# datvo06/MSAU

Measured on AMD Instinct MI355X. Metric: chargrid tiles/sec (train fwd+bwd), 336x256x64 3-stage MSAU, higher is better.
Workload: dtype bf16; 1 GPU; configs[1]: one-hot chargrid 336x256x64, 3-stage MSAU (featRoot 8, 4 scales, res_depth 2), batch 16/GPU, fwd+masked-CE+bwd+clip+Adam; global_batch=16, parallelism=dp1, graph=False

## Files before the change

### include/msau_hip.h

```cpp
#ifndef MSAU_HIP_H
#define MSAU_HIP_H

#include <stdint.h>

#ifdef __cplusplus
extern "C" {
#endif

typedef enum { MSAU_F32 = 0, MSAU_BF16 = 1 } msau_dtype;

typedef enum {
    MSAU_OK = 0,
    MSAU_ERR_ARG = -1,
    MSAU_ERR_LDS = -2,
    MSAU_ERR_HIP = -3
} msau_status;

const char* msau_last_error(void);
int msau_version(void);
const char* msau_source_hash(void);
int msau_sizeof(int which);
int msau_lds_pixel_stride(int raw_bytes, int esz, int c8_per_chunk, int read_stride);
int msau_lds_wrow_stride(int nks, int esz);

// ... 120 lines not shown
    int32_t KH, KW, dil, pad_t, pad_l, stride;
    int32_t flags;
    const void* x1;
    const void* x2;
    const void* g;
    float* slabs;
    int32_t nslabs;
} msau_wgrad_desc;

typedef struct {
    int32_t cch, nchunks;
    int32_t kext;
    int32_t max_slabs;
    int64_t slab_bytes;
    int32_t lean;
    int32_t reserved;
} msau_wgrad_geom;

int msau_wgrad_geometry(int dtype, const msau_wgrad_desc* d, msau_wgrad_geom* out);
int msau_conv2d_wgrad(void* stream, int dtype, const msau_wgrad_desc* d);
int msau_wgrad_route(int dtype, const msau_wgrad_desc* d, int32_t info[8]);
int msau_conv2d_wgrad_groupable(int dtype, const msau_wgrad_desc* a, const msau_wgrad_desc* b);
int msau_conv2d_wgrad_group(void* stream, int dtype, const msau_wgrad_desc* const* ds, int n);

typedef struct {
    int64_t src_off;
    int64_t dst_off;
    int32_t kind;
    int32_t dim0, dim1;
    int32_t KH, KW;
    int32_t row_is_dim0;
    int32_t flip;
    int32_t row_off;
    int32_t rows_real;
    int32_t rows_pad;
    int32_t k1_real, k1_store, k2_real, k2_store;
    int32_t cch, nchunks, kchunk;
    int32_t dtype;
} msau_pack_entry;

int msau_pack_params(void* stream, const float* flat_params, void* pack_arena,
                     const msau_pack_entry* table_dev, int n_entries, int max_elems_per_entry);

typedef struct {
    int64_t slab_off;
    int64_t w_off;
// ... 282 lines not shown
```

### msau_amd/_lib.py

```python
from __future__ import annotations

import ctypes as C
import os

HERE = os.path.dirname(os.path.abspath(__file__))
LIB_PATH = os.environ.get("MSAU_HIP_LIB", os.path.join(HERE, "libmsau_hip.so"))

F32, BF16 = 0, 1
OPTIM_ADAM, OPTIM_RMSPROP, OPTIM_MOMENTUM, OPTIM_MAX_SKIP = 0, 1, 2, 8
COST_CE, COST_FOCAL, COST_DICE = 0, 1, 2

CONV_RELU_IN, CONV_RELU_OUT, CONV_ADD, CONV_ACCUM, CONV_MASK_A, CONV_MASK_B, CONV_HEAD, CONV_DOUT = 1, 2, 4, 8, 16, 32, 64, 128
CONV_LRN, CONV_POOL, CONV_IDS, CONV_OWNER, CONV_NCHW, CONV_WGRAD, CONV_ELU = 256, 512, 1024, 2048, 4096, 8192, 32768
CONV_EXTENT = 65536

i32, i64, vp, f32 = C.c_int32, C.c_int64, C.c_void_p, C.c_float


class ConvDesc(C.Structure):
    _fields_ = [(n, i32) for n in ("B", "Hin", "Win", "Hout", "Wout", "C1", "C2", "Cout", "KH", "KW", "dil",
                                   "pad_t", "pad_l", "stride", "ups", "flags")] + \
               [(n, vp) for n in ("x1", "x2", "wpack", "bias", "add", "mask_a", "mask_b", "y", "head_probs", "head_argmax")] + \
               [("head_classes", i32), ("flags2", i32), ("y2", vp), ("mask_b2", vp)] + \
               [("lrn_alpha_over_n", f32), ("lrn_beta", f32), ("lrn_k", f32), ("reserved0", i32), ("pool_y", vp), ("pool_idx", vp)] + \
# ... 117 lines not shown
    "msau_conv2d": (C.c_int, [vp, C.c_int, C.POINTER(ConvDesc)]),
    "msau_conv2d_rider_slabs": (C.c_int, [C.c_int, C.POINTER(ConvDesc)]),
    "msau_attn_proj_bwd": (C.c_int, [vp, C.c_int, C.POINTER(AttnProjBwdArgs)]),
    "msau_dgrad2_1x1": (C.c_int, [vp, C.c_int, C.POINTER(Dgrad2Args)]),
    "msau_conv2d_launch_info": (C.c_int, [C.c_int, C.POINTER(ConvDesc), C.POINTER(i32)]),
    "msau_conv_pair_applicable": (C.c_int, [C.c_int, C.POINTER(ConvPairDesc)]),
    "msau_conv_pair": (C.c_int, [vp, C.c_int, C.POINTER(ConvPairDesc)]),
    "msau_conv_pair_bits_bytes": (C.c_int64, [C.c_int, C.POINTER(ConvPairDesc)]),
    "msau_conv_pair_instance": (C.c_int, [C.c_int, C.POINTER(ConvPairDesc)]),
    "msau_conv_pair_wgrad_slabs": (C.c_int, [C.c_int, C.POINTER(ConvPairDesc)]),
    "msau_owner_slabs": (C.c_int, [C.POINTER(WgradDesc)]),
    "msau_comm_available": (C.c_int, []),
    "msau_comm_unique_id": (C.c_int, [vp, C.c_int]),
    "msau_comm_init": (C.c_int, [C.POINTER(vp), C.c_int, C.c_int, vp, C.c_int]),
    "msau_comm_destroy": (C.c_int, [vp]),
    "msau_allreduce_bucket": (C.c_int, [vp, vp, vp, C.c_int64]),
    "msau_run_ops_dp": (C.c_int, [vp, vp, vp, C.POINTER(Op), C.c_int, C.c_int]),
    "msau_reload_env": (None, []),
    "msau_wgrad_geometry": (C.c_int, [C.c_int, C.POINTER(WgradDesc), C.POINTER(WgradGeom)]),
    "msau_conv2d_wgrad": (C.c_int, [vp, C.c_int, C.POINTER(WgradDesc)]),
    "msau_wgrad_route": (C.c_int, [C.c_int, C.POINTER(WgradDesc), C.POINTER(i32)]),
    "msau_conv2d_wgrad_groupable": (C.c_int, [C.c_int, C.POINTER(WgradDesc), C.POINTER(WgradDesc)]),
    "msau_conv2d_wgrad_group": (C.c_int, [vp, C.c_int, C.POINTER(C.POINTER(WgradDesc)), C.c_int]),
    "msau_pack_params": (C.c_int, [vp, vp, vp, vp, C.c_int, C.c_int]),
    "msau_wgrad_reduce": (C.c_int, [vp, vp, vp, vp, C.c_int, C.c_int]),
    "msau_channel_sum": (C.c_int, [vp, C.c_int, vp, i64, C.c_int, vp, C.c_int]),
    "msau_nchw_to_nhwc": (C.c_int, [vp, C.c_int, vp, vp] + [C.c_int] * 5),
    "msau_nhwc_to_nchw": (C.c_int, [vp, C.c_int, vp, vp] + [C.c_int] * 5),
    "msau_nchw_grad_to_nhwc": (C.c_int, [vp, C.c_int, vp, vp] + [C.c_int] * 6),
    "msau_lrn_fwd": (C.c_int, [vp, C.c_int, vp, vp, i64, C.c_int, C.c_int, C.c_int, f32, f32, f32]),
    "msau_lrn_bwd": (C.c_int, [vp, C.c_int, vp, vp, vp, i64, C.c_int, C.c_int, C.c_int, f32, f32, f32]),
    "msau_maxpool2x2_fwd": (C.c_int, [vp, C.c_int, vp, vp, vp] + [C.c_int] * 4),
    "msau_maxpool2x2_bwd": (C.c_int, [vp, C.c_int, vp, vp, vp, vp] + [C.c_int] * 5),
    "msau_selfattn_fwd": (C.c_int, [vp, C.c_int, vp, vp, vp, vp, vp, vp] + [C.c_int] * 4),
    "msau_selfattn_bwd": (C.c_int, [vp, C.c_int, vp, vp, vp, vp, vp, vp, vp, vp, vp] + [C.c_int] * 4),
    "msau_maxpool2x2_bwd_ext": (C.c_int, [vp, C.c_int, vp, vp, vp, vp] + [C.c_int] * 5 + [vp]),
    "msau_selfattn_fwd_ext": (C.c_int, [vp, C.c_int, vp, vp, vp, vp, vp, vp] + [C.c_int] * 4 + [vp, C.c_int]),
    "msau_selfattn_bwd_ext": (C.c_int, [vp, C.c_int, vp, vp, vp, vp, vp, vp, vp, vp, vp] + [C.c_int] * 4 + [vp, C.c_int]),
    "msau_selfattn_route": (C.c_int, [C.c_int] * 4),
    "msau_extent_copy": (C.c_int, [vp, vp, vp] + [C.c_int] * 5 + [vp]),
    "msau_label_counts": (C.c_int, [vp, vp, vp, C.c_int, i64]),
    "msau_label_counts_split": (C.c_int, [vp, vp, vp, C.c_int, i64, C.c_int]),
    "msau_ce_ws_floats": (i64, [i64]),
    "msau_ce_multi_ws_floats": (i64, [i64]),
    "msau_masked_ce_multi": (C.c_int, [vp, C.c_int, vp, vp, vp, vp, vp, vp, vp, vp, C.c_int, i64, C.c_int, C.c_int, f32, C.c_int]),
    "msau_masked_ce": (C.c_int, [vp, C.c_int, vp, vp, vp, vp, vp, vp, C.c_int, i64, C.c_int, C.c_int, f32]),
# ... 180 lines not shown
```

### msau_amd/csrc/conv_wgrad.hip

```cpp
#include "msau_common.h"

namespace {

struct WGeom {
    int esz, taps, cch, nchunks, kreal, kextc, NKT, NKW, CTN, compact, slice;
    int TIH, TIW, PSx, PSg, x_bytes, g_bytes, tab_bytes, total;
};

inline int pix_stride(int c, int esz) {
    int ps = c * esz;
    if (((ps >> 4) & 1) == 0) ps += 16;
    return ps;
}

int wgrad_geom(int dtype, const msau_wgrad_desc* d, WGeom* out) {
    MSAU_CHECK_ARG(dtype == MSAU_F32 || dtype == MSAU_BF16, "wgrad: bad dtype");
    const int Cin = d->C1 + d->C2;
    MSAU_CHECK_ARG(Cin > 0 && Cin % 8 == 0 && d->Cout > 0 && d->Cout % 8 == 0 && d->Cout <= 1024, "wgrad: bad channels");
    MSAU_CHECK_ARG(d->KH >= 1 && d->KW >= 1 && d->KH <= 7 && d->KW <= 7 && d->dil >= 1 && (d->stride == 1 || d->stride == 2), "wgrad: bad kernel");
    WGeom g;
    g.esz = dtype == MSAU_F32 ? 4 : 2;
    g.taps = d->KH * d->KW;
    g.compact = d->stride == 1 && d->dil >= 16 && g.taps > 1;
    g.slice = g.esz == 4 ? (g.compact ? 32 : 64) : 128;
// ... 324 lines not shown
}

extern "C" int msau_conv2d_wgrad_groupable(int dtype, const msau_wgrad_desc* a, const msau_wgrad_desc* b) {
    if (!a || !b) return 0;
    WGeom g;
    WRoute r;
    return wgrad_route(dtype, a, &g, &r) == 0 && wgrad_groupable(r, a, b);
}

extern "C" int msau_conv2d_wgrad_group(void* stream, int dtype, const msau_wgrad_desc* const* ds, int n) {
    MSAU_CHECK_ARG(ds && n >= 1 && n <= 4, "wgrad_group: 1..4 launches");
    WGeom g;
    WRoute r;
    int rc = 0;
    for (int i = 0; i < n; ++i) {
        MSAU_CHECK_ARG(ds[i] && ds[i]->x1 && ds[i]->g && ds[i]->slabs && (ds[i]->C2 == 0 || ds[i]->x2), "wgrad_group: null pointer");
        if (i == 0 && n > 1) rc = wgrad_route(dtype, ds[0], &g, &r);
        MSAU_CHECK_ARG(i == 0 || (rc == 0 && wgrad_groupable(r, ds[0], ds[i])), "wgrad_group: launch %d differs in shape from launch 0", i);
    }
    if (n == 1) return msau_conv2d_wgrad(stream, dtype, ds[0]);
    if ((rc = wgrad_check_nslabs(ds[0], r))) return rc;
    return msau_wgrad_lean_launch(static_cast<hipStream_t>(stream), dtype, ds, n, &r);
}
```

### msau_amd/csrc/msau_common.h

```cpp
#pragma once
#include <hip/hip_runtime.h>
#include <stdint.h>
#include <stdio.h>
#include <stdarg.h>
#include "../../include/msau_hip.h"

typedef __bf16 bf16_t;
typedef __bf16 bf16x8 __attribute__((ext_vector_type(8)));
typedef __bf16 bf16x4 __attribute__((ext_vector_type(4)));
typedef float f32x4 __attribute__((ext_vector_type(4)));
typedef float f32x8 __attribute__((ext_vector_type(8)));

#define MSAU_LDS_LIMIT (160 * 1024)

int msau_set_error(int code, const char* fmt, ...);

constexpr int kFwd1 = MSAU_PAIR_RELU_IN | MSAU_PAIR_RELU_MID, kFwd2 = MSAU_CONV_ADD | MSAU_CONV_RELU_OUT;
constexpr int kBwd1 = MSAU_PAIR_MASK_MID, kBwd2 = MSAU_CONV_MASK_A | MSAU_CONV_ADD;
constexpr int kPairFwdRiders = MSAU_PAIR_COUPLE, kPairBwdRiders = MSAU_PAIR_LRN_BWD | MSAU_PAIR_WGRAD1 | MSAU_PAIR_DCOUPLE;
constexpr int kPairRiders = MSAU_PAIR_TILES | kPairFwdRiders | kPairBwdRiders;
enum { PAIR_NONE = 0, PAIR_TILE = 1, PAIR_ROWS = 2 };
enum { PAIR_FWD = 1, PAIR_BWD = 2 };
static inline int msau_pair_direction(const msau_conv_pair_desc* d) {
    const int f1 = d->flags1 & ~kPairRiders;
// ... 11 lines not shown
int msau_rowpair_case(int dtype, const msau_conv_pair_desc* d);
void msau_rowpair_split(const msau_conv_pair_desc* d, PairRoute* r);
int msau_rowpair_launch(hipStream_t s, const msau_conv_pair_desc* d, const PairRoute* r);
int msau_ownerconv_takes(int dtype, const msau_conv_desc* d);
int msau_ownerconv_fwd(hipStream_t s, int dtype, const msau_conv_desc* d);
int msau_rowconv_case(int dtype, const msau_conv_desc* d, int kchunk, int rows);
int msau_rowconv_launch(hipStream_t s, const msau_conv_desc* d, int kchunk, int rows, int inst);
int msau_rowconv_workgroups(const msau_conv_desc* d, int inst);
int msau_conv_chunked_case(int dtype, const msau_conv_desc* d, int cch, int nchunks, int CT);
int msau_conv_chunked_launch(hipStream_t s, int dtype, const msau_conv_desc* d, int kchunk, int nchunks, int CT, int which);
int msau_conv_lean_case(int dtype, const msau_conv_desc* d, int nchunks, int CT);
int msau_conv_lean_launch(hipStream_t s, int dtype, const msau_conv_desc* d, int kchunk, int CT, int which);
int msau_firstconv_takes(int dtype, const msau_conv_desc* d);
int msau_firstconv_launch(hipStream_t s, int dtype, const msau_conv_desc* d, int real_channels);
enum { WF_NONE = 0, WF_TILE = 1, WF_LEAN = 2, WF_SPECIAL = 3, WF_IN64 = 4, WF_IN64_IDS = 5, WF_ROWS = 6, WF_OWNER = 7 };
struct WRoute {
    int family, inst;
    int CTN, NKW, slices;
    int cch, nchunks, kextc;
    int tiles_x, tiles_y, ntiles;
};
int msau_wgrad_lean_case(int dtype, const msau_wgrad_desc* d, int cch, int kextc);
int msau_wgrad_lean_launch(hipStream_t s, int dtype, const msau_wgrad_desc* const* ds, int n, const WRoute* r);
int msau_rowwgrad_case(int dtype, const msau_wgrad_desc* d, int cch, int nchunks, int kextc);
int msau_rowwgrad_launch(hipStream_t s, const msau_wgrad_desc* d, int inst);
int msau_ownerconv_wgrad_case(int dtype, const msau_wgrad_desc* d, int cch, int nchunks, int kextc);
int msau_ownerconv_wgrad_launch(hipStream_t s, int dtype, const msau_wgrad_desc* d, const WRoute* r);

#define MSAU_CHECK_ARG(cond, ...)                                   \
    do {                                                            \
        if (!(cond)) return msau_set_error(MSAU_ERR_ARG, __VA_ARGS__); \
    } while (0)

#define MSAU_CHECK_LAUNCH(name)                                                         \
    do {                                                                                \
        hipError_t e__ = hipGetLastError();                                             \
        if (e__ != hipSuccess)                                                          \
            return msau_set_error(MSAU_ERR_HIP, "%s: %s", name, hipGetErrorString(e__)); \
    } while (0)

static inline int64_t cdiv64(int64_t a, int64_t b) { return (a + b - 1) / b; }
static inline int cdiv(int a, int b) { return (a + b - 1) / b; }
static inline int roundup(int a, int b) { return cdiv(a, b) * b; }

constexpr int kThreads = 256;

// ... 94 lines not shown
```

### msau_amd/csrc/sequence.hip

```cpp
#include "msau_common.h"

#include <cstdlib>
#include <utility>
#include <vector>

static int run_one_raw(void* stream, const msau_op& o, int i);

namespace {
struct ProbePair { hipEvent_t a, b; };
thread_local std::vector<ProbePair> g_probe_pool;
thread_local size_t g_probe_used = 0;
}

static int run_one(void* stream, const msau_op& o_in, int i) {
    if (!(o_in.kind & MSAU_OP_PROBE)) return run_one_raw(stream, o_in, i);
    msau_op o = o_in;
    o.kind &= ~MSAU_OP_PROBE;
    if (g_probe_used == g_probe_pool.size()) {
        ProbePair p;
        if (hipEventCreate(&p.a) != hipSuccess || hipEventCreate(&p.b) != hipSuccess)
            return msau_set_error(MSAU_ERR_HIP, "run_ops: cannot create probe events");
        g_probe_pool.push_back(p);
    }
    ProbePair& p = g_probe_pool[g_probe_used++];
// ... 65 lines not shown
        std::vector<hipEvent_t>& pl = sys ? pool_sys : pool;
        size_t& u = sys ? used_sys : used;
        if (u == pl.size()) {
            hipEvent_t e;
            hipError_t err = hipEventCreateWithFlags(&e, hipEventDisableTiming | (sys || fence_all ? 0u : hipEventDisableSystemFence));
            if (err != hipSuccess) return msau_set_error(MSAU_ERR_HIP, "run_ops_overlap: event: %s", hipGetErrorString(err));
            pl.push_back(e);
        }
        *ev = pl[u++];
        return 0;
    };
    auto next_event = [&](hipEvent_t* ev) -> int { return next_event_of(ev, false); };
    static const int fork_every = std::getenv("MSAU_FORK_EVERY") ? atoi(std::getenv("MSAU_FORK_EVERY")) : 6;
    std::vector<std::pair<msau_op, int>> pending;
    bool any_side = false;
    auto flush = [&]() -> int {
        if (pending.empty()) return 0;
        hipEvent_t ev;
        int rc = next_event(&ev);
        if (rc) return rc;
        if (hipEventRecord(ev, ms) != hipSuccess || hipStreamWaitEvent(ss, ev, 0) != hipSuccess)
            return msau_set_error(MSAU_ERR_HIP, "run_ops_overlap: fork failed");
        static const bool group_off = std::getenv("MSAU_WGRAD_GROUP") && std::getenv("MSAU_WGRAD_GROUP")[0] == '0';
        std::vector<char> done(pending.size(), 0);
        for (size_t i = 0; i < pending.size(); ++i) {
            if (done[i]) continue;
            const msau_op& o = pending[i].first;
            if (!group_off && o.kind == MSAU_OP_WGRAD) {
                const msau_wgrad_desc* ds[4] = {static_cast<const msau_wgrad_desc*>(o.args), nullptr, nullptr, nullptr};
                int n = 1;
                for (size_t j = i + 1; j < pending.size() && n < 4; ++j) {
                    const msau_op& p = pending[j].first;
                    if (done[j] || p.kind != MSAU_OP_WGRAD || p.dtype != o.dtype) continue;
                    if (!msau_conv2d_wgrad_groupable(o.dtype, ds[0], static_cast<const msau_wgrad_desc*>(p.args))) continue;
                    ds[n++] = static_cast<const msau_wgrad_desc*>(p.args);
                    done[j] = 1;
                }
                if (n > 1) {
                    rc = msau_conv2d_wgrad_group(side_stream, o.dtype, ds, n);
                    if (rc) return rc;
                    continue;
                }
            }
            rc = run_one(side_stream, o, pending[i].second);
            if (rc) return rc;
        }
        pending.clear();
        any_side = true;
        return 0;
    };
// ... 130 lines not shown
```

### msau_amd/csrc/wgrad_lean.hip

```cpp
#include "msau_common.h"
#include <cstdlib>

namespace {

struct WLeanArgs {
    msau_wgrad_desc d;
    int kextc, nchunks;
    int tiles_x, tiles_y, ntiles;
    unsigned mag_tx, mag_ty;
};

constexpr int kWGroup = 4;
struct WLeanMulti { WLeanArgs a[kWGroup]; };

#define WL_ABS 0x40000000
#ifndef MSAU_WPS_MAX
#define MSAU_WPS_MAX 10
#endif

typedef __attribute__((address_space(3))) bf16x4* lds_v4;

template <typename T, int C8, int CO8, int KS, int DIL = 1, int STRIDE = 1>
struct WLeanCfg {
    static constexpr int ESZ = (int)sizeof(T);
// ... 2 lines not shown
    static constexpr int QS = NMAP ? 4 : 8;
    static constexpr int HI = NMAP ? 8 : 4;
    static constexpr int PSX = NMAP ? lds_pixel_stride(C8 * 8 * ESZ, ESZ, C8, STRIDE) : (((C8 * 8 * ESZ / 16) % 2 == 0) ? C8 * 8 * ESZ + 16 : C8 * 8 * ESZ);
    static constexpr int PSG = NMAP ? lds_pixel_stride(CO8 * 8 * ESZ, ESZ, CO8, 1) : (((CO8 * 8 * ESZ / 16) % 2 == 0) ? CO8 * 8 * ESZ + 16 : CO8 * 8 * ESZ);
    static constexpr int KREAL = KS * KS * C8 * 8;
    static constexpr int KEXT = ((KREAL + 8 + 15) / 16) * 16;
    static constexpr int NKT = KEXT / 16;
    static constexpr int NKW = (NKT + 3) / 4;
    static constexpr int CTN = (CO8 + 1) / 2;
    static constexpr int X_BYTES = ((TI * TI * PSX + 15) / 16) * 16;
    static constexpr int G_BYTES = 256 * PSG;
    static constexpr bool PS = ESZ == 2 && NKT * CTN <= MSAU_WPS_MAX;
#ifndef MSAU_WGRAD_W2
#define MSAU_WGRAD_W2 1
#endif
    static constexpr bool W2 = MSAU_WGRAD_W2 && ESZ == 2 && !PS;
    static constexpr int NTH = W2 ? 512 : 256;
    static constexpr int RED_BYTES = PS ? 4 * NKT * CTN * 1024 : 0;
    static constexpr int TILE_BYTES = X_BYTES + G_BYTES + 64;
    static constexpr int LDS = TILE_BYTES > RED_BYTES ? TILE_BYTES : RED_BYTES;
};

template <typename T, int C8, int CO8, int KS, int DIL = 1, int STRIDE = 1>
__global__ __launch_bounds__((WLeanCfg<T, C8, CO8, KS, DIL, STRIDE>::NTH)) void wgrad_lean_kernel(const WLeanMulti m) {
    const WLeanArgs a = m.a[blockIdx.z];
    using Cfg = WLeanCfg<T, C8, CO8, KS, DIL, STRIDE>;
    typedef typename Vec8<T>::type V8;
    constexpr int ESZ = Cfg::ESZ, TI = Cfg::TI, PSX = Cfg::PSX, PSG = Cfg::PSG, NKT = Cfg::NKT, NKW = Cfg::NKW, CTN = Cfg::CTN;
    extern __shared__ __align__(16) unsigned char smem[];
    unsigned char* lds_x = smem;
    unsigned char* lds_g = smem + Cfg::X_BYTES;
    constexpr int ONES = Cfg::X_BYTES + Cfg::G_BYTES;

    const msau_wgrad_desc& d = a.d;
    constexpr int NTH = Cfg::NTH;
    const int tid = threadIdx.x, lane = tid & 63;
    const int wave = __builtin_amdgcn_readfirstlane((tid >> 6) & 3);
    const int wset = Cfg::W2 ? __builtin_amdgcn_readfirstlane(tid >> 8) : 0;
    const int li = lane & 15, lg = lane >> 4;
    const int chunk = blockIdx.y;
    const bool relu_in = d.flags & MSAU_CONV_RELU_IN;

    const int c0 = chunk * C8 * 8;
    const bool second = d.C2 != 0 && c0 >= d.C1;
    const char* xsrc = static_cast<const char*>(second ? d.x2 : d.x1);
    const int Cx = second ? d.C2 : d.C1;
    const int cb = (second ? c0 - d.C1 : c0) * ESZ;
    const int in_px = Cx * ESZ, in_row = d.Win * in_px;
    const int g_px = d.Cout * ESZ, g_row = d.Wout * g_px;

    if (tid < 8) reinterpret_cast<T*>(smem + ONES)[tid] = (T)(tid == 0 ? 1.0f : 0.0f);

    constexpr bool PS = Cfg::PS;
    constexpr int NACC = PS ? NKT : NKW;
    int coloff[NACC];
#pragma unroll
    for (int i = 0; i < NACC; ++i) {
        const int nkt = PS ? i : wave + 4 * i;
        const int k = nkt * 16 + (sizeof(T) == 2 ? (li & 3) * 4 : (li >> 2) * 4);
        int off;
        if (!PS && nkt >= NKT) off = WL_ABS | (ONES + 4 * ESZ);
        else if (k < Cfg::KREAL) {
            const int tap = k / (C8 * 8), c = k - tap * (C8 * 8);
// ... 29 lines not shown
                const int idx = tid + it * NTH;
                xr[it] = zero8<T>();
                if ((it + 1) * NTH <= NITEMS || idx < NITEMS) {
                    const int pix = idx / C8, cg = idx - pix * C8;
                    const int iy = pix / TI, ix = pix - iy * TI;
                    const int vy = vy0 + iy, vx = vx0 + ix;
                    if ((unsigned)vy < (unsigned)d.Hin && (unsigned)vx < (unsigned)d.Win)
                        xr[it] = *reinterpret_cast<const V8*>(base + (unsigned)(vy * in_row + vx * in_px + cg * 8 * ESZ));
                }
            }
        }
        {
            const char* base = static_cast<const char*>(d.g) + (long long)b * d.Hout * g_row;
#pragma unroll
            for (int it = 0; it < NITG; ++it) {
                const int idx = tid + it * NTH;
                const int m = idx / CO8, cg = idx - m * CO8;
                const int oy = oy0 + (m >> 4), ox = ox0 + (m & 15);
                gr[it] = zero8<T>();
                if (idx < 256 * CO8 && oy < d.Hout && ox < d.Wout) gr[it] = *reinterpret_cast<const V8*>(base + (unsigned)(oy * g_row + ox * g_px + cg * 8 * ESZ));
            }
        }
    };
    if (PIPE && (int)blockIdx.x < a.ntiles) issue_loads(blockIdx.x);

    for (int tile = blockIdx.x; tile < a.ntiles; tile += gridDim.x) {
        __syncthreads();
        if (!PIPE) issue_loads(tile);
        {
            constexpr int NITEMS = TI * TI * C8;
#pragma unroll
            for (int it = 0; it < NITX; ++it) {
                const int idx = tid + it * NTH;
                if ((it + 1) * NTH <= NITEMS || idx < NITEMS) {
                    const int pix = idx / C8, cg = idx - pix * C8;
                    V8 v = xr[it];
                    if (relu_in) v = relu8<T>(v);
                    *reinterpret_cast<V8*>(lds_x + pix * PSX + cg * 8 * ESZ) = v;
                }
            }
#pragma unroll
            for (int it = 0; it < NITG; ++it) {
                const int idx = tid + it * NTH;
                const int m = idx / CO8, cg = idx - m * CO8;
                if (idx < 256 * CO8) *reinterpret_cast<V8*>(lds_g + m * PSG + cg * 8 * ESZ) = gr[it];
            }
        }
        __syncthreads();
        if (PIPE && tile + (int)gridDim.x < a.ntiles) issue_loads(tile + gridDim.x);

        if constexpr (PS) {
            const int q = li >> 2, p = li & 3;
#pragma unroll
            for (int bb = 0; bb < 2; ++bb) {
                const int blk = wave * 2 + bb;
                const int row = blk * 2 + (lg >> 1), col = (lg & 1) * Cfg::QS + q;
                const unsigned char* ga = lds_g + (row * 16 + col) * PSG + 4 * p * 2;
                bf16x8 afrag[CTN];
#pragma unroll
                for (int ct = 0; ct < CTN; ++ct) {
                    bf16x4 lo = __builtin_amdgcn_ds_read_tr16_b64_v4bf16((lds_v4)(ga + ct * 32));
                    bf16x4 hi = __builtin_amdgcn_ds_read_tr16_b64_v4bf16((lds_v4)(ga + Cfg::HI * PSG + ct * 32));
                    afrag[ct] = __builtin_shufflevector(lo, hi, 0, 1, 2, 3, 4, 5, 6, 7);
                }
                const int pb0 = (row * STRIDE * TI + col * STRIDE) * PSX;
#pragma unroll
                for (int i = 0; i < NKT; ++i) {
                    const int e = coloff[i];
                    const bool abs_ok = (i + 1) * 16 > Cfg::KREAL;
                    const int o0 = (abs_ok && (e & WL_ABS)) ? (e & ~WL_ABS) : pb0 + e;
                    const int o1 = (abs_ok && (e & WL_ABS)) ? (e & ~WL_ABS) : pb0 + Cfg::HI * STRIDE * PSX + e;
                    bf16x4 lo = __builtin_amdgcn_ds_read_tr16_b64_v4bf16((lds_v4)(smem + o0));
// ... 33 lines not shown
                    for (int ct = 0; ct < CTN; ++ct)
                        acc[i][ct] = __builtin_amdgcn_mfma_f32_16x16x32_bf16(afrag[ct], bfrag, acc[i][ct], 0, 0, 0);
                }
            }
        } else {
            for (int step = 0; step < 64; ++step) {
                const int m = step * 4 + lg;
                float afrag[CTN];
#pragma unroll
                for (int ct = 0; ct < CTN; ++ct) afrag[ct] = *reinterpret_cast<const float*>(lds_g + m * PSG + (ct * 16 + li) * 4);
                const int pb = ((m >> 4) * STRIDE * TI + (m & 15) * STRIDE) * PSX;
#pragma unroll
                for (int i = 0; i < NKW; ++i) {
                    const int e = coloff[i];
                    const float bv = *reinterpret_cast<const float*>(smem + ((e & WL_ABS) ? (e & ~WL_ABS) : pb + e));
#pragma unroll
                    for (int ct = 0; ct < CTN; ++ct)
                        acc[i][ct] = __builtin_amdgcn_mfma_f32_16x16x4f32(afrag[ct], bv, acc[i][ct], 0, 0, 0);
                }
            }
        }
    }

    float* slab = d.slabs + ((size_t)blockIdx.x * a.nchunks + chunk) * d.Cout * a.kextc;
    if constexpr (PS) {
        __syncthreads();
        f32x4* red = reinterpret_cast<f32x4*>(smem);
#pragma unroll
        for (int i = 0; i < NKT; ++i)
#pragma unroll
            for (int ct = 0; ct < CTN; ++ct) red[((wave * NKT + i) * CTN + ct) * 64 + lane] = acc[i][ct];
        __syncthreads();
#pragma unroll
        for (int ii = 0; ii < NKW; ++ii) {
            const int nkt = wave + 4 * ii;
            if (nkt >= NKT) continue;
#pragma unroll
            for (int ct = 0; ct < CTN; ++ct) {
                f32x4 v = red[((0 * NKT + nkt) * CTN + ct) * 64 + lane];
#pragma unroll
                for (int w = 1; w < 4; ++w) v += red[((w * NKT + nkt) * CTN + ct) * 64 + lane];
#pragma unroll
                for (int j = 0; j < 4; ++j) {
                    const int co = ct * 16 + lg * 4 + j;
                    if (co < d.Cout) slab[(size_t)co * a.kextc + nkt * 16 + li] = v[j];
                }
            }
        }
        return;
    }
    if constexpr (Cfg::W2) {
        constexpr int PER = Cfg::TILE_BYTES / (4 * CTN * 1024) < 1 ? 1 : Cfg::TILE_BYTES / (4 * CTN * 1024);
        f32x4* red = reinterpret_cast<f32x4*>(smem);
        for (int i0 = 0; i0 < NKW; i0 += PER) {
            __syncthreads();
            if (wset == 1) {
#pragma unroll
                for (int i = 0; i < NKW; ++i)
                    if (i >= i0 && i < i0 + PER)
#pragma unroll
                        for (int ct = 0; ct < CTN; ++ct) red[((wave * PER + (i - i0)) * CTN + ct) * 64 + lane] = acc[i][ct];
            }
            __syncthreads();
            if (wset == 0) {
#pragma unroll
                for (int i = 0; i < NKW; ++i)
                    if (i >= i0 && i < i0 + PER)
#pragma unroll
                        for (int ct = 0; ct < CTN; ++ct) acc[i][ct] += red[((wave * PER + (i - i0)) * CTN + ct) * 64 + lane];
            }
        }
        if (wset == 1) return;
    }
#pragma unroll
    for (int i = 0; i < NKW; ++i) {
        const int nkt = wave + 4 * i;
        if (nkt >= NKT) continue;
#pragma unroll
        for (int ct = 0; ct < CTN; ++ct)
#pragma unroll
            for (int j = 0; j < 4; ++j) {
                const int co = ct * 16 + lg * 4 + j;
                if (co < d.Cout) slab[(size_t)co * a.kextc + nkt * 16 + li] = acc[i][ct][j];
            }
    }
}


struct WIn64 {
    static constexpr int PSX = 64 * 2 + 32, PSG = 8 * 2 + 32, TG = 18;
    static constexpr int X_BYTES = 256 * PSX, G_BYTES = TG * TG * PSG;
    static constexpr int ZERO = X_BYTES + G_BYTES;
    static constexpr int TILE_BYTES = ZERO + 64;
    static constexpr int RED_BYTES = 4 * 10 * 1024;
    static constexpr int LDS = TILE_BYTES > RED_BYTES ? TILE_BYTES : RED_BYTES;
};

template <bool IDS>
__global__ __launch_bounds__(256) void wgrad_in64_kernel(const WLeanArgs a) {
    typedef bf16_t T;
    typedef Vec8<T>::type V8;
    constexpr int PSX = WIn64::PSX, PSG = WIn64::PSG, TG = WIn64::TG;
    extern __shared__ __align__(16) unsigned char smem[];
    unsigned char* lds_x = smem;
    unsigned char* lds_g = smem + WIn64::X_BYTES;
    const msau_wgrad_desc& d = a.d;
    const int tid = threadIdx.x, lane = tid & 63;
    const int wave = __builtin_amdgcn_readfirstlane(tid >> 6);
// ... 199 lines not shown
#define WLEAN_TABLE(X)                                                                                                          \
    WLEAN_SHAPES(X, 1) WLEAN_SHAPES(X, 3) X(WF_LEAN, 8, 8, 1, 1, 1, 1) X(WF_LEAN, 8, 8, 3, 1, 1, 0) X(WF_LEAN, 1, 1, 4, 1, 1, 1)   \
    X(WF_SPECIAL, 1, 2, 3, 2, 1, 1) X(WF_SPECIAL, 2, 4, 3, 4, 1, 1) X(WF_SPECIAL, 4, 8, 3, 8, 1, 0)                             \
    X(WF_SPECIAL, 1, 2, 3, 1, 2, 1) X(WF_SPECIAL, 2, 4, 3, 1, 2, 1) X(WF_SPECIAL, 4, 8, 3, 1, 2, 0)                             \
    X(WF_IN64, 8, 1, 3, 1, 1, 0)

template <typename T>
int wlean_instance(int id, int kextc, hipStream_t s, const WLeanMulti* m, int n) {
    switch (id) {
#define WLEAN_ROW(FAM, C8, CO8, KS, DIL, STRIDE, F32)                                                                           \
        case wlean_id(FAM, C8, CO8, KS, DIL, STRIDE):                                                                           \
            if constexpr (FAM == WF_IN64) {                                                                                     \
                if (sizeof(T) == 2 && kextc == 592) return m ? launch_wgrad_in64(s, m->a[0]) : 1;                                \
            } else if constexpr (F32 || sizeof(T) == 2) {                                                                       \
                if (WLeanCfg<T, C8, CO8, KS, DIL, STRIDE>::KEXT == kextc) return m ? launch_wlean<T, C8, CO8, KS, DIL, STRIDE>(s, *m, n) : 1; \
            }                                                                                                                   \
            break;
        WLEAN_TABLE(WLEAN_ROW)
#undef WLEAN_ROW
    }
    return m ? msau_set_error(MSAU_ERR_ARG, "wgrad_lean: no instance %#x with k extent %d", id, kextc) : 0;
}

bool wlean_in64(int dtype, const msau_wgrad_desc* d, int cch) {
    static const bool in64_off = std::getenv("MSAU_WGRAD_IN64") && std::getenv("MSAU_WGRAD_IN64")[0] == '0';
    return !in64_off && dtype == MSAU_BF16 && d->stride == 1 && d->dil == 1 && d->KH == 3 && cch == 64 && d->Cout == 8 &&
           d->pad_t <= 2 && d->pad_l <= 2;
}

}

int msau_wgrad_lean_case(int dtype, const msau_wgrad_desc* d, int cch, int kextc) {
    if (d->KH != d->KW || d->dil > 8) return 0;
    const bool special = d->stride != 1 || d->dil != 1;
    if (special) {
        if (d->C2 || cch != d->C1 || d->pad_t != d->dil || d->pad_l != d->dil) return 0;
    } else {
        if (d->Hin != d->Hout || d->Win != d->Wout || d->pad_t < 0 || d->pad_l < 0 || d->pad_t >= d->KH || d->pad_l >= d->KW) return 0;
    }
    const int esz = dtype == MSAU_F32 ? 4 : 2;
    if ((int64_t)d->Hin * d->Win * (d->C1 > d->C2 ? d->C1 : d->C2) * esz >= (1ll << 31)) return 0;
    if ((int64_t)d->Hout * d->Wout * d->Cout * esz >= (1ll << 31)) return 0;
    const int tx = cdiv(d->Wout, 16), ty = cdiv(d->Hout, 16);
    if ((int64_t)d->B * tx * ty >= (1 << 20) || tx >= 4096 || ty >= 4096) return 0;
    const int fam = special ? WF_SPECIAL : wlean_in64(dtype, d, cch) ? WF_IN64 : WF_LEAN;
    const int id = wlean_id(fam, cch / 8, d->Cout / 8, d->KH, d->dil, d->stride);
    return (dtype == MSAU_F32 ? wlean_instance<float>(id, kextc, nullptr, nullptr, 0) : wlean_instance<bf16_t>(id, kextc, nullptr, nullptr, 0)) ? id : 0;
}

int msau_wgrad_lean_launch(hipStream_t s, int dtype, const msau_wgrad_desc* const* ds, int n, const WRoute* r) {
    MSAU_CHECK_ARG(n >= 1 && n <= ((r->inst & 7) == WF_IN64 ? 1 : kWGroup), "wgrad_lean: %d launches in one grid", n);
    WLeanMulti m;
    for (int i = 0; i < n; ++i) {
        WLeanArgs& a = m.a[i];
        a.d = *ds[i];
        a.kextc = r->kextc; a.nchunks = r->nchunks;
        a.tiles_x = r->tiles_x; a.tiles_y = r->tiles_y; a.ntiles = r->ntiles;
        a.mag_tx = (unsigned)((0x100000000ull + a.tiles_x - 1) / a.tiles_x);
        a.mag_ty = (unsigned)((0x100000000ull + a.tiles_y - 1) / a.tiles_y);
    }
    for (int i = n; i < kWGroup; ++i) m.a[i] = m.a[0];
    return dtype == MSAU_F32 ? wlean_instance<float>(r->inst, r->kextc, s, &m, n) : wlean_instance<bf16_t>(r->inst, r->kextc, s, &m, n);
}
```

Measured before the change: 5776 tiles/s.

## Batch wgrad lean layers of one occupancy class into a single persistent task kernel

Adds a task-list kernel that runs weight-gradient computations for up to 16 lean-route layers in one launch. Layers are grouped by an occupancy class derived from register and LDS limits, then sorted by per-slab work length, and each block dispatches to the right templated body through a switch. The goal is to cut per-layer launch overhead and fill the GPU better when each small layer alone uses fewer blocks than there are CUs. In exchange the kernel argument struct is larger, the dynamic LDS is sized for the largest member, and the switch may affect code size and register allocation.

```diff
diff --git a/include/msau_hip.h b/include/msau_hip.h
--- a/include/msau_hip.h
+++ b/include/msau_hip.h
@@ -166,6 +166,8 @@
 int msau_wgrad_route(int dtype, const msau_wgrad_desc* d, int32_t info[8]);
 int msau_conv2d_wgrad_groupable(int dtype, const msau_wgrad_desc* a, const msau_wgrad_desc* b);
 int msau_conv2d_wgrad_group(void* stream, int dtype, const msau_wgrad_desc* const* ds, int n);
+int msau_conv2d_wgrad_task_class(int dtype, const msau_wgrad_desc* d);
+int msau_conv2d_wgrad_tasks(void* stream, int dtype, const msau_wgrad_desc* const* ds, int n);
 
 typedef struct {
     int64_t src_off;
diff --git a/msau_amd/_lib.py b/msau_amd/_lib.py
--- a/msau_amd/_lib.py
+++ b/msau_amd/_lib.py
@@ -163,6 +163,8 @@
     "msau_wgrad_route": (C.c_int, [C.c_int, C.POINTER(WgradDesc), C.POINTER(i32)]),
     "msau_conv2d_wgrad_groupable": (C.c_int, [C.c_int, C.POINTER(WgradDesc), C.POINTER(WgradDesc)]),
     "msau_conv2d_wgrad_group": (C.c_int, [vp, C.c_int, C.POINTER(C.POINTER(WgradDesc)), C.c_int]),
+    "msau_conv2d_wgrad_task_class": (C.c_int, [C.c_int, C.POINTER(WgradDesc)]),
+    "msau_conv2d_wgrad_tasks": (C.c_int, [vp, C.c_int, C.POINTER(C.POINTER(WgradDesc)), C.c_int]),
     "msau_pack_params": (C.c_int, [vp, vp, vp, vp, C.c_int, C.c_int]),
     "msau_wgrad_reduce": (C.c_int, [vp, vp, vp, vp, C.c_int, C.c_int]),
     "msau_channel_sum": (C.c_int, [vp, C.c_int, vp, i64, C.c_int, vp, C.c_int]),
diff --git a/msau_amd/csrc/conv_wgrad.hip b/msau_amd/csrc/conv_wgrad.hip
--- a/msau_amd/csrc/conv_wgrad.hip
+++ b/msau_amd/csrc/conv_wgrad.hip
@@ -370,3 +370,50 @@
     if ((rc = wgrad_check_nslabs(ds[0], r))) return rc;
     return msau_wgrad_lean_launch(static_cast<hipStream_t>(stream), dtype, ds, n, &r);
 }
+
+
+namespace {
+int device_cus() {
+    static const int cus = [] {
+        int dev = 0, n = 0;
+        if (hipGetDevice(&dev) != hipSuccess || hipDeviceGetAttribute(&n, hipDeviceAttributeMultiprocessorCount, dev) != hipSuccess || n <= 0) {
+            (void)hipGetLastError();
+            n = 256;
+        }
+        return n;
+    }();
+    return cus;
+}
+
+int wgrad_task_class(int dtype, const msau_wgrad_desc* d, const WRoute& r) {
+    if (r.family != WF_LEAN && r.family != WF_SPECIAL) return 0;
+    if (d->nslabs < 1 || (int64_t)d->nslabs * r.nchunks > device_cus()) return 0;
+    return msau_wgrad_lean_task_class(dtype, &r);
+}
+}
+
+extern "C" int msau_conv2d_wgrad_task_class(int dtype, const msau_wgrad_desc* d) {
+    if (!d) return 0;
+    WGeom g;
+    WRoute r;
+    return wgrad_route(dtype, d, &g, &r) == 0 ? wgrad_task_class(dtype, d, r) : 0;
+}
+
+extern "C" int msau_conv2d_wgrad_tasks(void* stream, int dtype, const msau_wgrad_desc* const* ds, int n) {
+    MSAU_CHECK_ARG(ds && n >= 2 && n <= 16, "wgrad_tasks: 2..16 launches");
+    WGeom g;
+    WRoute rs[16];
+    int cls = 0;
+    for (int i = 0; i < n; ++i) {
+        const msau_wgrad_desc* d = ds[i];
+        MSAU_CHECK_ARG(d && d->x1 && d->g && d->slabs && (d->C2 == 0 || d->x2), "wgrad_tasks: null pointer");
+        int rc = wgrad_route(dtype, d, &g, &rs[i]);
+        if (rc) return rc;
+        if ((rc = wgrad_check_nslabs(d, rs[i]))) return rc;
+        const int c = wgrad_task_class(dtype, d, rs[i]);
+        MSAU_CHECK_ARG(c != 0, "wgrad_tasks: launch %d has no task class", i);
+        MSAU_CHECK_ARG(i == 0 || c == cls, "wgrad_tasks: launch %d is of task class %d, launch 0 of %d", i, c, cls);
+        cls = c;
+    }
+    return msau_wgrad_lean_tasks(static_cast<hipStream_t>(stream), dtype, cls, ds, rs, n);
+}
diff --git a/msau_amd/csrc/msau_common.h b/msau_amd/csrc/msau_common.h
--- a/msau_amd/csrc/msau_common.h
+++ b/msau_amd/csrc/msau_common.h
@@ -57,6 +57,8 @@
 };
 int msau_wgrad_lean_case(int dtype, const msau_wgrad_desc* d, int cch, int kextc);
 int msau_wgrad_lean_launch(hipStream_t s, int dtype, const msau_wgrad_desc* const* ds, int n, const WRoute* r);
+int msau_wgrad_lean_task_class(int dtype, const WRoute* r);
+int msau_wgrad_lean_tasks(hipStream_t s, int dtype, int cls, const msau_wgrad_desc* const* ds, const WRoute* rs, int n);
 int msau_rowwgrad_case(int dtype, const msau_wgrad_desc* d, int cch, int nchunks, int kextc);
 int msau_rowwgrad_launch(hipStream_t s, const msau_wgrad_desc* d, int inst);
 int msau_ownerconv_wgrad_case(int dtype, const msau_wgrad_desc* d, int cch, int nchunks, int kextc);
diff --git a/msau_amd/csrc/sequence.hip b/msau_amd/csrc/sequence.hip
--- a/msau_amd/csrc/sequence.hip
+++ b/msau_amd/csrc/sequence.hip
@@ -111,10 +111,32 @@
         if (hipEventRecord(ev, ms) != hipSuccess || hipStreamWaitEvent(ss, ev, 0) != hipSuccess)
             return msau_set_error(MSAU_ERR_HIP, "run_ops_overlap: fork failed");
         static const bool group_off = std::getenv("MSAU_WGRAD_GROUP") && std::getenv("MSAU_WGRAD_GROUP")[0] == '0';
+        static const bool tasks_off = std::getenv("MSAU_WGRAD_TASKS") && std::getenv("MSAU_WGRAD_TASKS")[0] == '0';
         std::vector<char> done(pending.size(), 0);
+        std::vector<int> cls(pending.size(), 0);
+        if (!tasks_off && pending.size() > 1)
+            for (size_t i = 0; i < pending.size(); ++i)
+                if (pending[i].first.kind == MSAU_OP_WGRAD)
+                    cls[i] = msau_conv2d_wgrad_task_class(pending[i].first.dtype, static_cast<const msau_wgrad_desc*>(pending[i].first.args));
         for (size_t i = 0; i < pending.size(); ++i) {
             if (done[i]) continue;
             const msau_op& o = pending[i].first;
+            if (cls[i]) {
+                const msau_wgrad_desc* ts[16] = {static_cast<const msau_wgrad_desc*>(o.args)};
+                size_t at[16];
+                int n = 1;
+                for (size_t j = i + 1; j < pending.size() && n < 16; ++j) {
+                    if (done[j] || cls[j] != cls[i] || pending[j].first.dtype != o.dtype) continue;
+                    at[n] = j;
+                    ts[n++] = static_cast<const msau_wgrad_desc*>(pending[j].first.args);
+                }
+                if (n > 1) {
+                    rc = msau_conv2d_wgrad_tasks(side_stream, o.dtype, ts, n);
+                    if (rc) return rc;
+                    for (int k = 1; k < n; ++k) done[at[k]] = 1;
+                    continue;
+                }
+            }
             if (!group_off && o.kind == MSAU_OP_WGRAD) {
                 const msau_wgrad_desc* ds[4] = {static_cast<const msau_wgrad_desc*>(o.args), nullptr, nullptr, nullptr};
                 int n = 1;
diff --git a/msau_amd/csrc/wgrad_lean.hip b/msau_amd/csrc/wgrad_lean.hip
--- a/msau_amd/csrc/wgrad_lean.hip
+++ b/msau_amd/csrc/wgrad_lean.hip
@@ -48,8 +48,7 @@
 };
 
 template <typename T, int C8, int CO8, int KS, int DIL = 1, int STRIDE = 1>
-__global__ __launch_bounds__((WLeanCfg<T, C8, CO8, KS, DIL, STRIDE>::NTH)) void wgrad_lean_kernel(const WLeanMulti m) {
-    const WLeanArgs a = m.a[blockIdx.z];
+__device__ __forceinline__ void wgrad_lean_body(const WLeanArgs& a, const unsigned slab_i, const unsigned nslab, const int chunk) {
     using Cfg = WLeanCfg<T, C8, CO8, KS, DIL, STRIDE>;
     typedef typename Vec8<T>::type V8;
     constexpr int ESZ = Cfg::ESZ, TI = Cfg::TI, PSX = Cfg::PSX, PSG = Cfg::PSG, NKT = Cfg::NKT, NKW = Cfg::NKW, CTN = Cfg::CTN;
@@ -64,7 +63,6 @@
     const int wave = __builtin_amdgcn_readfirstlane((tid >> 6) & 3);
     const int wset = Cfg::W2 ? __builtin_amdgcn_readfirstlane(tid >> 8) : 0;
     const int li = lane & 15, lg = lane >> 4;
-    const int chunk = blockIdx.y;
     const bool relu_in = d.flags & MSAU_CONV_RELU_IN;
 
     const int c0 = chunk * C8 * 8;
@@ -140,9 +138,9 @@
             }
         }
     };
-    if (PIPE && (int)blockIdx.x < a.ntiles) issue_loads(blockIdx.x);
-
-    for (int tile = blockIdx.x; tile < a.ntiles; tile += gridDim.x) {
+    if (PIPE && (int)slab_i < a.ntiles) issue_loads(slab_i);
+
+    for (int tile = slab_i; tile < a.ntiles; tile += nslab) {
         __syncthreads();
         if (!PIPE) issue_loads(tile);
         {
@@ -165,7 +163,7 @@
             }
         }
         __syncthreads();
-        if (PIPE && tile + (int)gridDim.x < a.ntiles) issue_loads(tile + gridDim.x);
+        if (PIPE && tile + (int)nslab < a.ntiles) issue_loads(tile + nslab);
 
         if constexpr (PS) {
             const int q = li >> 2, p = li & 3;
@@ -245,7 +243,7 @@
         }
     }
 
-    float* slab = d.slabs + ((size_t)blockIdx.x * a.nchunks + chunk) * d.Cout * a.kextc;
+    float* slab = d.slabs + ((size_t)slab_i * a.nchunks + chunk) * d.Cout * a.kextc;
     if constexpr (PS) {
         __syncthreads();
         f32x4* red = reinterpret_cast<f32x4*>(smem);
@@ -270,8 +268,7 @@
                 }
             }
         }
-        return;
-    }
+    } else {
     if constexpr (Cfg::W2) {
         constexpr int PER = Cfg::TILE_BYTES / (4 * CTN * 1024) < 1 ? 1 : Cfg::TILE_BYTES / (4 * CTN * 1024);
         f32x4* red = reinterpret_cast<f32x4*>(smem);
@@ -293,20 +290,28 @@
                         for (int ct = 0; ct < CTN; ++ct) acc[i][ct] += red[((wave * PER + (i - i0)) * CTN + ct) * 64 + lane];
             }
         }
-        if (wset == 1) return;
-    }
-#pragma unroll
-    for (int i = 0; i < NKW; ++i) {
-        const int nkt = wave + 4 * i;
-        if (nkt >= NKT) continue;
-#pragma unroll
-        for (int ct = 0; ct < CTN; ++ct)
-#pragma unroll
-            for (int j = 0; j < 4; ++j) {
-                const int co = ct * 16 + lg * 4 + j;
-                if (co < d.Cout) slab[(size_t)co * a.kextc + nkt * 16 + li] = acc[i][ct][j];
-            }
-    }
+    }
+    if (wset == 0) {
+#pragma unroll
+        for (int i = 0; i < NKW; ++i) {
+            const int nkt = wave + 4 * i;
+            if (nkt >= NKT) continue;
+#pragma unroll
+            for (int ct = 0; ct < CTN; ++ct)
+#pragma unroll
+                for (int j = 0; j < 4; ++j) {
+                    const int co = ct * 16 + lg * 4 + j;
+                    if (co < d.Cout) slab[(size_t)co * a.kextc + nkt * 16 + li] = acc[i][ct][j];
+                }
+        }
+    }
+    }
+}
+
+template <typename T, int C8, int CO8, int KS, int DIL = 1, int STRIDE = 1>
+__global__ __launch_bounds__((WLeanCfg<T, C8, CO8, KS, DIL, STRIDE>::NTH)) void wgrad_lean_kernel(const WLeanMulti m) {
+    const WLeanArgs a = m.a[blockIdx.z];
+    wgrad_lean_body<T, C8, CO8, KS, DIL, STRIDE>(a, blockIdx.x, gridDim.x, blockIdx.y);
 }
 
 
@@ -552,6 +557,118 @@
     return m ? msau_set_error(MSAU_ERR_ARG, "wgrad_lean: no instance %#x with k extent %d", id, kextc) : 0;
 }
 
+#define WLEAN_WAVES(W)                                                              \
+    W(1, 1, 1, 1, 1, 8, 4) W(1, 2, 1, 1, 1, 8, 4) W(2, 1, 1, 1, 1, 8, 3) W(2, 2, 1, 1, 1, 8, 3) W(2, 4, 1, 1, 1, 4, 2)           \
+    W(4, 2, 1, 1, 1, 5, 2) W(4, 4, 1, 1, 1, 4, 2) W(8, 1, 1, 1, 1, 4, 3) W(4, 8, 1, 1, 1, 4, 2) W(8, 4, 1, 1, 1, 3, 2)           \
+    W(1, 1, 3, 1, 1, 7, 7) W(1, 2, 3, 1, 1, 5, 6) W(2, 1, 3, 1, 1, 4, 5) W(2, 2, 3, 1, 1, 4, 4) W(2, 4, 3, 1, 1, 4, 3)           \
+    W(4, 2, 3, 1, 1, 4, 3) W(4, 4, 3, 1, 1, 3, 2) W(8, 1, 3, 1, 1, 3, 2) W(4, 8, 3, 1, 1, 2, 1) W(8, 4, 3, 1, 1, 2, 1)           \
+    W(8, 8, 1, 1, 1, 4, 2) W(8, 8, 3, 1, 1, 2, 0) W(1, 1, 4, 1, 1, 4, 7)                                                         \
+    W(1, 2, 3, 2, 1, 5, 7) W(2, 4, 3, 4, 1, 4, 3) W(4, 8, 3, 8, 1, 2, 0) W(1, 2, 3, 1, 2, 4, 4) W(2, 4, 3, 1, 2, 3, 2)           \
+    W(4, 8, 3, 1, 2, 2, 0)
+constexpr int wlean_waves(int esz, int c8, int co8, int ks, int dil, int stride) {
+    switch (wlean_id(0, c8, co8, ks, dil, stride)) {
+#define WLEAN_WAVES_ROW(C8, CO8, KS, DIL, STRIDE, WB, WF) case wlean_id(0, C8, CO8, KS, DIL, STRIDE): return esz == 2 ? WB : WF;
+        WLEAN_WAVES(WLEAN_WAVES_ROW)
+#undef WLEAN_WAVES_ROW
+    }
+    return 0;
+}
+template <typename T, int C8, int CO8, int KS, int DIL, int STRIDE>
+constexpr int wlean_class() {
+    using Cfg = WLeanCfg<T, C8, CO8, KS, DIL, STRIDE>;
+    const int by_regs = wlean_waves((int)sizeof(T), C8, CO8, KS, DIL, STRIDE);
+    const int by_lds = MSAU_LDS_LIMIT / Cfg::LDS * (Cfg::NTH / 256);
+    return (Cfg::NTH == 512 ? 8 : 0) + (by_regs < by_lds ? by_regs : by_lds);
+}
+template <typename T, int CLS, int FAM, int C8, int CO8, int KS, int DIL, int STRIDE, int F32>
+constexpr bool wlean_in_class() {
+    if constexpr (FAM != WF_IN64 && (F32 || sizeof(T) == 2)) return wlean_class<T, C8, CO8, KS, DIL, STRIDE>() == CLS;
+    else return false;
+}
+template <typename T, int CLS>
+constexpr bool wlean_class_used() {
+    bool any = false;
+#define WLEAN_ROW(FAM, C8, CO8, KS, DIL, STRIDE, F32) any = any || wlean_in_class<T, CLS, FAM, C8, CO8, KS, DIL, STRIDE, F32>();
+    WLEAN_TABLE(WLEAN_ROW)
+#undef WLEAN_ROW
+    return any;
+}
+
+constexpr int kWTasks = 16;
+struct WTaskList {
+    WLeanArgs a[kWTasks];
+    int inst[kWTasks];
+    int first[kWTasks + 1];
+};
+static_assert(sizeof(WTaskList) <= 4096, "the task list is a kernel argument");
+
+template <typename T, int CLS>
+__global__ __launch_bounds__((CLS > 8 ? 512 : 256)) __attribute__((amdgpu_waves_per_eu((CLS - 1) % 8 + 1 < 8 ? (CLS - 1) % 8 + 1 : 1)))
+void wgrad_tasks_kernel(const WTaskList tl) {
+    const int t = blockIdx.x;
+    int layer = 0;
+#pragma unroll
+    for (int i = 1; i < kWTasks; ++i) layer += t >= tl.first[i];
+    const WLeanArgs a = tl.a[layer];
+    const int local = t - tl.first[layer];
+    const int chunk = local / a.d.nslabs, slab_i = local - chunk * a.d.nslabs;
+    switch (tl.inst[layer]) {
+#define WLEAN_ROW(FAM, C8, CO8, KS, DIL, STRIDE, F32)                                                                           \
+        case wlean_id(FAM, C8, CO8, KS, DIL, STRIDE):                                                                           \
+            if constexpr (wlean_in_class<T, CLS, FAM, C8, CO8, KS, DIL, STRIDE, F32>())                                          \
+                wgrad_lean_body<T, C8, CO8, KS, DIL, STRIDE>(a, slab_i, a.d.nslabs, chunk);                                      \
+            break;
+        WLEAN_TABLE(WLEAN_ROW)
+#undef WLEAN_ROW
+    }
+}
+
+template <typename T>
+int wlean_task_info(int id, int kextc, int* lds) {
+    switch (id) {
+#define WLEAN_ROW(FAM, C8, CO8, KS, DIL, STRIDE, F32)                                                                           \
+        case wlean_id(FAM, C8, CO8, KS, DIL, STRIDE):                                                                           \
+            if constexpr (FAM != WF_IN64 && (F32 || sizeof(T) == 2)) {                                                          \
+                if (WLeanCfg<T, C8, CO8, KS, DIL, STRIDE>::KEXT != kextc) return 0;                                              \
+                if (lds) *lds = WLeanCfg<T, C8, CO8, KS, DIL, STRIDE>::LDS;                                                      \
+                return wlean_class<T, C8, CO8, KS, DIL, STRIDE>();                                                               \
+            }                                                                                                                   \
+            break;
+        WLEAN_TABLE(WLEAN_ROW)
+#undef WLEAN_ROW
+    }
+    return 0;
+}
+
+template <typename T, int CLS>
+int launch_wtasks(hipStream_t s, const WTaskList& tl, int grid, int lds) {
+    if constexpr (!wlean_class_used<T, CLS>()) {
+        return msau_set_error(MSAU_ERR_ARG, "wgrad_tasks: no instance in class %d", CLS);
+    } else {
+        static bool attr_set = false;
+        if (!attr_set) {
+            hipError_t e = hipFuncSetAttribute(reinterpret_cast<const void*>(&wgrad_tasks_kernel<T, CLS>),
+                                               hipFuncAttributeMaxDynamicSharedMemorySize, MSAU_LDS_LIMIT);
+            if (e != hipSuccess) return msau_set_error(MSAU_ERR_HIP, "wgrad_tasks: hipFuncSetAttribute: %s", hipGetErrorString(e));
+            attr_set = true;
+        }
+        hipLaunchKernelGGL((wgrad_tasks_kernel<T, CLS>), dim3(grid), dim3(CLS > 8 ? 512 : 256), lds, s, tl);
+        MSAU_CHECK_LAUNCH("wgrad_tasks_kernel");
+        return 0;
+    }
+}
+
+template <typename T>
+int launch_wtasks_class(int cls, hipStream_t s, const WTaskList& tl, int grid, int lds) {
+    switch (cls) {
+#define WTASK_CLASS(N) case N: return launch_wtasks<T, N>(s, tl, grid, lds);
+        WTASK_CLASS(1) WTASK_CLASS(2) WTASK_CLASS(3) WTASK_CLASS(4) WTASK_CLASS(5) WTASK_CLASS(6) WTASK_CLASS(7) WTASK_CLASS(8)
+        WTASK_CLASS(9) WTASK_CLASS(10) WTASK_CLASS(11) WTASK_CLASS(12) WTASK_CLASS(13) WTASK_CLASS(14) WTASK_CLASS(15) WTASK_CLASS(16)
+#undef WTASK_CLASS
+    }
+    return msau_set_error(MSAU_ERR_ARG, "wgrad_tasks: bad class %d", cls);
+}
+
 bool wlean_in64(int dtype, const msau_wgrad_desc* d, int cch) {
     static const bool in64_off = std::getenv("MSAU_WGRAD_IN64") && std::getenv("MSAU_WGRAD_IN64")[0] == '0';
     return !in64_off && dtype == MSAU_BF16 && d->stride == 1 && d->dil == 1 && d->KH == 3 && cch == 64 && d->Cout == 8 &&
@@ -578,17 +695,50 @@
     return (dtype == MSAU_F32 ? wlean_instance<float>(id, kextc, nullptr, nullptr, 0) : wlean_instance<bf16_t>(id, kextc, nullptr, nullptr, 0)) ? id : 0;
 }
 
+static void wlean_fill(WLeanArgs* a, const msau_wgrad_desc* d, const WRoute* r) {
+    a->d = *d;
+    a->kextc = r->kextc; a->nchunks = r->nchunks;
+    a->tiles_x = r->tiles_x; a->tiles_y = r->tiles_y; a->ntiles = r->ntiles;
+    a->mag_tx = (unsigned)((0x100000000ull + a->tiles_x - 1) / a->tiles_x);
+    a->mag_ty = (unsigned)((0x100000000ull + a->tiles_y - 1) / a->tiles_y);
+}
+
 int msau_wgrad_lean_launch(hipStream_t s, int dtype, const msau_wgrad_desc* const* ds, int n, const WRoute* r) {
     MSAU_CHECK_ARG(n >= 1 && n <= ((r->inst & 7) == WF_IN64 ? 1 : kWGroup), "wgrad_lean: %d launches in one grid", n);
     WLeanMulti m;
-    for (int i = 0; i < n; ++i) {
-        WLeanArgs& a = m.a[i];
-        a.d = *ds[i];
-        a.kextc = r->kextc; a.nchunks = r->nchunks;
-        a.tiles_x = r->tiles_x; a.tiles_y = r->tiles_y; a.ntiles = r->ntiles;
-        a.mag_tx = (unsigned)((0x100000000ull + a.tiles_x - 1) / a.tiles_x);
-        a.mag_ty = (unsigned)((0x100000000ull + a.tiles_y - 1) / a.tiles_y);
-    }
+    for (int i = 0; i < n; ++i) wlean_fill(&m.a[i], ds[i], r);
     for (int i = n; i < kWGroup; ++i) m.a[i] = m.a[0];
     return dtype == MSAU_F32 ? wlean_instance<float>(r->inst, r->kextc, s, &m, n) : wlean_instance<bf16_t>(r->inst, r->kextc, s, &m, n);
 }
+
+
+int msau_wgrad_lean_task_class(int dtype, const WRoute* r) {
+    return dtype == MSAU_F32 ? wlean_task_info<float>(r->inst, r->kextc, nullptr) : wlean_task_info<bf16_t>(r->inst, r->kextc, nullptr);
+}
+
+int msau_wgrad_lean_tasks(hipStream_t s, int dtype, int cls, const msau_wgrad_desc* const* ds, const WRoute* rs, int n) {
+    MSAU_CHECK_ARG(n >= 1 && n <= kWTasks, "wgrad_tasks: %d layers in one list", n);
+    int order[kWTasks];
+    for (int i = 0; i < n; ++i) {
+        const int len = cdiv(rs[i].ntiles, ds[i]->nslabs);
+        int j = i;
+        for (; j > 0 && cdiv(rs[order[j - 1]].ntiles, ds[order[j - 1]]->nslabs) < len; --j) order[j] = order[j - 1];
+        order[j] = i;
+    }
+    WTaskList tl;
+    int grid = 0, lds = 0;
+    for (int k = 0; k < n; ++k) {
+        const int i = order[k];
+        int l = 0;
+        const int c = dtype == MSAU_F32 ? wlean_task_info<float>(rs[i].inst, rs[i].kextc, &l) : wlean_task_info<bf16_t>(rs[i].inst, rs[i].kextc, &l);
+        MSAU_CHECK_ARG(c == cls, "wgrad_tasks: layer %d is of task class %d, not %d", i, c, cls);
+        wlean_fill(&tl.a[k], ds[i], &rs[i]);
+        tl.inst[k] = rs[i].inst;
+        tl.first[k] = grid;
+        grid += ds[i]->nslabs * rs[i].nchunks;
+        if (l > lds) lds = l;
+    }
+    for (int k = n; k < kWTasks; ++k) { tl.a[k] = tl.a[0]; tl.inst[k] = 0; }
+    for (int k = n; k <= kWTasks; ++k) tl.first[k] = grid;
+    return dtype == MSAU_F32 ? launch_wtasks_class<float>(cls, s, tl, grid, lds) : launch_wtasks_class<bf16_t>(cls, s, tl, grid, lds);
+}
```

New measurement: 5789 tiles/s (median of 3 runs). Within noise of the previous version (+0.2%).
